# ut-amrl/vision_slam_frontend

Measured on AMD Instinct MI355X. Metric: stereo frames/s (640x480, 2000 kp/frame), higher is better.
Workload: dtype u8

## Files before the change

include/vsf.h:

```cpp
#ifndef VSF_H_
#define VSF_H_

#include <stddef.h>
#include <stdint.h>

#ifdef __cplusplus
extern "C" {
#endif

#define VSF_VERSION 2
#define VSF_DESC_BYTES 32
#define VSF_MAX_LEVELS 64

typedef enum {
  VSF_OK = 0,
  VSF_ERR_INVALID_ARG = 1,
  VSF_ERR_CAPACITY = 2,
  VSF_ERR_HIP = 3,
  VSF_ERR_UNSUPPORTED = 4,
  VSF_ERR_NO_DEVICE = 5
} vsf_status;

typedef struct {
  float x, y;
// ... 12 lines not shown
typedef struct {
  int32_t nfeatures;
  float scale_factor;
  int32_t nlevels;
  int32_t edge_threshold;
  int32_t first_level;
  int32_t wta_k;
  int32_t score_type;
  int32_t patch_size;
  int32_t fast_threshold;
  int32_t blur_sse2;
  int32_t fast_detector_threshold;
  int32_t fast_detector_nms;
  uint32_t ratio_num;
  uint32_t ratio_shift;
  int32_t width, height;
  int32_t max_images;
  int32_t max_keypoints;
  int32_t residual_order;
} vsf_params;

typedef struct vsf_ctx vsf_ctx;

vsf_status vsf_params_default(vsf_params* p, int width, int height, int max_images);
vsf_status vsf_params_set_ratio(vsf_params* p, float nn_match_ratio);

vsf_status vsf_create(const vsf_params* p, int device, vsf_ctx** out);
void vsf_destroy(vsf_ctx* ctx);
const char* vsf_status_string(vsf_status s);
int vsf_last_hip_error(const vsf_ctx* ctx);
vsf_status vsf_get_params(const vsf_ctx* ctx, vsf_params* out);
vsf_status vsf_set_stream(vsf_ctx* ctx, void* hip_stream);
vsf_status vsf_set_lanes(vsf_ctx* ctx, int lanes);
vsf_status vsf_set_pipeline(vsf_ctx* ctx, int on);
vsf_status vsf_set_input_event(vsf_ctx* ctx, void* hip_event);
vsf_status vsf_set_blur_overlap(vsf_ctx* ctx, int on);
vsf_status vsf_set_fast_resident(vsf_ctx* ctx, int waves);
vsf_status vsf_get_fast_resident(const vsf_ctx* ctx, int* waves);
vsf_status vsf_tune_fast_resident(vsf_ctx* ctx, const uint8_t* d_imgs, int n_images, size_t image_stride,
                                  size_t row_stride, vsf_keypoint* d_kp, uint8_t* d_desc, int32_t* d_counts,
                                  int samples, float* ms_grid, float* ms_resident);
typedef enum {
  VSF_OPT_FAST_BOTH_MAX = 0,
  VSF_OPT_SELECT_WIDE = 1,
  VSF_OPT_PYRAMID_FEW = 2,
  VSF_OPT_PYRAMID_CHAIN = 3,
  VSF_OPT_PYRAMID_ROWS = 4,
  VSF_OPT_SELECT_BIG_CLASS = 5,
  VSF_OPT_PIPE_AFTER_FAST = 6,
  VSF_OPT_PIPE_PRIORITY = 7,
  VSF_OPT_OBSERVE_THREAD = 8,
  VSF_OPT_PYRAMID_TAIL_MIN = 9,
  VSF_OPT_OBSERVE_COPY_THREAD = 10,
  VSF_OPT_COUNT = 11
} vsf_option;
vsf_status vsf_set_option(vsf_ctx* ctx, int option, int value);
vsf_status vsf_get_option(const vsf_ctx* ctx, int option, int* value);
vsf_status vsf_sync(vsf_ctx* ctx);
vsf_status vsf_reserve(vsf_ctx* ctx, int n_frames, int n_pairs);

vsf_status vsf_level_info(const vsf_ctx* ctx, int level, int* w, int* h, float* scale, int* nfeatures);

#define VSF_COMM_ID_BYTES 128
typedef struct vsf_comm vsf_comm;
vsf_status vsf_comm_unique_id(uint8_t* id);
vsf_status vsf_comm_create(vsf_ctx* ctx, const uint8_t* id, int rank, int world, vsf_comm** out);
void vsf_comm_destroy(vsf_comm* comm);
vsf_status vsf_comm_info(const vsf_comm* comm, int* rank, int* world, int* rccl_version);
vsf_status vsf_allgather_dev(vsf_ctx* ctx, vsf_comm* comm, const void* d_send, void* d_recv, size_t bytes_per_rank);
vsf_status vsf_gather_payload_dev(vsf_ctx* ctx, vsf_comm* comm, const uint8_t* d_send, size_t bytes, uint8_t* d_recv,
                                  size_t recv_stride, int root);


vsf_status vsf_extract(vsf_ctx* ctx, const uint8_t* img, int w, int h, size_t stride, vsf_keypoint* kp_out,
                       uint8_t* desc_out, int cap, int* n_out);
vsf_status vsf_extract_pair(vsf_ctx* ctx, const uint8_t* img0, const uint8_t* img1, int w, int h, size_t stride,
                            vsf_keypoint* kp0, uint8_t* desc0, int* n0, vsf_keypoint* kp1, uint8_t* desc1, int* n1,
                            int cap);
vsf_status vsf_fast_detect(vsf_ctx* ctx, const uint8_t* img, int w, int h, size_t stride, int threshold, int nms,
                           vsf_keypoint* kp_out, int cap, int* n_out);
vsf_status vsf_knn2_hamming(vsf_ctx* ctx, const uint8_t* q, int nq, const uint8_t* t, int nt, int32_t* idx2,
                            int32_t* dist2);
vsf_status vsf_get_matches(vsf_ctx* ctx, const uint8_t* q, int nq, const uint8_t* t, int nt, vsf_dmatch* out,
                           int cap, int* n_out);

vsf_status vsf_get_matches_multi(vsf_ctx* ctx, const uint8_t* const* q, const int* nq, int n_sets, const uint8_t* t,
                                 int nt, vsf_dmatch* out, int cap_per_set, int* n_out);


vsf_status vsf_extract_batch_dev(vsf_ctx* ctx, const uint8_t* d_imgs, int n_images, size_t image_stride,
                                 size_t row_stride, vsf_keypoint* d_kp, uint8_t* d_desc, int32_t* d_counts);
vsf_status vsf_match_batch_dev(vsf_ctx* ctx, const uint8_t* d_desc, const int32_t* d_counts, size_t set_stride,
                               const int32_t* d_q_set, const int32_t* d_t_set, int n_pairs, int32_t* d_idx2,
                               int32_t* d_dist2, vsf_dmatch* d_matches, int32_t* d_nmatches);
vsf_status vsf_stereo_batch_dev(vsf_ctx* ctx, const uint8_t* d_imgs, int n_frames, size_t image_stride,
                                size_t row_stride, vsf_keypoint* d_kp, uint8_t* d_desc, int32_t* d_counts,
                                vsf_dmatch* d_matches, int32_t* d_nmatches);


vsf_status vsf_remove_ambig_stereo_batch_dev(vsf_ctx* ctx, const vsf_keypoint* d_kp, const uint8_t* d_desc,
                                             const vsf_dmatch* d_matches, const int32_t* d_nmatches, int n_frames,
                                             const float* F, float thr_in, const float* d_thr_override,
                                             float* d_means, float* d_thr, vsf_keypoint* d_kp_out,
                                             uint8_t* d_desc_out, int32_t* d_counts_out);
vsf_status vsf_feature_matches_batch_dev(vsf_ctx* ctx, const uint8_t* d_desc, const int32_t* d_counts,
                                         size_t set_stride, const int32_t* d_q_set, const int32_t* d_t_set,
                                         int n_pairs, float best_percent, uint64_t* d_pairs, int32_t* d_npairs);
// ... 96 lines not shown
```

vision_slam_frontend_amd/capi.py:

```python
from __future__ import annotations

import ctypes as C
from pathlib import Path

import numpy as np

_PKG = Path(__file__).resolve().parent
LIB_PATH = _PKG / "libvsf_hip.so"

KEYPOINT_DTYPE = np.dtype([("x", "<f4"), ("y", "<f4"), ("size", "<f4"), ("angle", "<f4"), ("response", "<f4"),
                           ("octave", "<i4"), ("class_id", "<i4")])
DMATCH_DTYPE = np.dtype([("queryIdx", "<i4"), ("trainIdx", "<i4"), ("imgIdx", "<i4"), ("distance", "<f4")])
VISION_FEATURE_DTYPE = np.dtype([("feature_idx", "<u8"), ("pixel", "<f4", (2,)), ("point3d", "<f4", (3,))])
FEATURE_MATCH_DTYPE = np.dtype([("feature_idx_initial", "<u8"), ("feature_idx_current", "<u8")])
assert VISION_FEATURE_DTYPE.itemsize == 28 and FEATURE_MATCH_DTYPE.itemsize == 16
DESC_BYTES = 32
PAYLOAD_MAGIC = 0x31465356

VSF_OK, VSF_ERR_INVALID_ARG, VSF_ERR_CAPACITY, VSF_ERR_HIP, VSF_ERR_UNSUPPORTED, VSF_ERR_NO_DEVICE = range(6)

EXPORTS = [
    "vsf_params_default", "vsf_params_set_ratio", "vsf_create", "vsf_destroy", "vsf_status_string",
    "vsf_last_hip_error", "vsf_get_params", "vsf_set_stream", "vsf_sync", "vsf_level_info", "vsf_extract",
    "vsf_fast_detect", "vsf_knn2_hamming", "vsf_get_matches", "vsf_extract_pair", "vsf_get_matches_multi", "vsf_extract_batch_dev", "vsf_match_batch_dev",
    "vsf_stereo_batch_dev", "vsf_set_lanes", "vsf_set_pipeline", "vsf_set_blur_overlap", "vsf_set_fast_resident", "vsf_get_fast_resident", "vsf_remove_ambig_stereo_batch_dev", "vsf_feature_matches_batch_dev", "vsf_bayer_bg_to_gray_batch_dev", "vsf_debug_level_image", "vsf_debug_fast_candidates", "vsf_debug_level_keypoints",
    "vsf_algorithmic_bytes_per_image", "vsf_pyramid_pixels", "vsf_profile_enable", "vsf_profile_read",
    "vsf_stage_name", "vsf_debug_retain_best", "vsf_debug_sort_trim", "vsf_stereo_residuals_batch_dev", "vsf_stereo_thresholds_dev",
    "vsf_stereo_filter_batch_dev", "vsf_vision_features_batch_dev", "vsf_packed_outputs_capacity",
    "vsf_pack_outputs_dev", "vsf_observe_capacity", "vsf_observe_stereo", "vsf_observe_submit", "vsf_observe_collect", "vsf_observe_reset",
    "vsf_observe_configure", "vsf_observe_collect_view", "vsf_observe_stats", "vsf_observe_poll", "vsf_debug_jpeg_serial",
    "vsf_jpeg_decode_gray_batch", "vsf_png_decode_gray_batch", "vsf_imdecode_gray_batch", "vsf_tune_fast_resident", "vsf_set_option", "vsf_get_option", "vsf_debug_inject_hip_error", "vsf_comm_unique_id", "vsf_comm_create", "vsf_comm_destroy", "vsf_comm_info",
    "vsf_allgather_dev", "vsf_gather_payload_dev", "vsf_reserve", "vsf_set_input_event",
]
(OPT_FAST_BOTH_MAX, OPT_SELECT_WIDE, OPT_PYRAMID_FEW, OPT_PYRAMID_CHAIN, OPT_PYRAMID_ROWS, OPT_SELECT_BIG_CLASS,
 OPT_PIPE_AFTER_FAST, OPT_PIPE_PRIORITY, OPT_OBSERVE_THREAD, OPT_PYRAMID_TAIL_MIN, OPT_OBSERVE_COPY_THREAD) = range(11)
STAGE_COUNT = 8


class VsfParams(C.Structure):
    _fields_ = [("nfeatures", C.c_int32), ("scale_factor", C.c_float), ("nlevels", C.c_int32),
                ("edge_threshold", C.c_int32), ("first_level", C.c_int32), ("wta_k", C.c_int32),
                ("score_type", C.c_int32), ("patch_size", C.c_int32), ("fast_threshold", C.c_int32),
                ("blur_sse2", C.c_int32), ("fast_detector_threshold", C.c_int32), ("fast_detector_nms", C.c_int32),
                ("ratio_num", C.c_uint32), ("ratio_shift", C.c_uint32), ("width", C.c_int32), ("height", C.c_int32),
                ("max_images", C.c_int32), ("max_keypoints", C.c_int32), ("residual_order", C.c_int32)]


class VsfCalibration(C.Structure):
    _fields_ = [("projection_left", C.c_float * 12), ("projection_right", C.c_float * 12),
                ("camera_matrix_left", C.c_float * 9), ("distortion_left", C.c_float * 5),
                ("fundamental", C.c_float * 9), ("triangulate_rows", C.c_int32)]

    def set(self, name: str, values) -> "VsfCalibration":
        arr = getattr(self, name)
        v = np.ascontiguousarray(values, np.float32).reshape(-1)
        assert len(v) == len(arr), name
        for i, x in enumerate(v):
            arr[i] = float(x)
        return self

    def get(self, name: str) -> np.ndarray:
        return np.array(list(getattr(self, name)), np.float32)


class VsfError(RuntimeError):
    def __init__(self, status: int, where: str, hip: int = 0):
        self.status = status
        msg = "%s: %s" % (where, lib().vsf_status_string(status).decode())
        if status == VSF_ERR_HIP:
            msg += " (hipError %d)" % hip
        super().__init__(msg)


_lib = None


def lib() -> C.CDLL:
    global _lib
    if _lib is None:
        if not LIB_PATH.exists():
            raise ImportError("%s is missing: run `python -c 'import __graft_entry__ as g; g.build()'` "
                              "(hipcc --offload-arch=gfx950). The product has no CPU fallback." % LIB_PATH)
        L = C.CDLL(str(LIB_PATH))
        vp, i32, sz, pp = C.c_void_p, C.c_int, C.c_size_t, C.POINTER(VsfParams)
        ip = C.POINTER(C.c_int)
        L.vsf_params_default.argtypes = [pp, i32, i32, i32]
        L.vsf_params_set_ratio.argtypes = [pp, C.c_float]
        L.vsf_create.argtypes = [pp, i32, C.POINTER(vp)]
# ... 515 lines not shown
```

vision_slam_frontend_amd/csrc/vsf_api.hip:

```cpp
#include <algorithm>
#include <cfloat>
#include <climits>
#include <cmath>
#include <cstdio>
#include <cstring>
#include <new>
#include <vector>

#include "vsf_ctx.h"

using namespace vsfi;

thread_local int vsf_tls_hip_error = 0;

namespace vsfi {

vsf_status alloc_devset(vsf_ctx* ctx, const Geometry& G, DevSet* ds, bool orb, int n_images) {
  VSF_HIP(upload(&ds->levels, G.levels));
  VSF_HIP(upload(&ds->units, G.units));
  VSF_HIP(upload(&ds->blur_mma_units, G.blur_mma_units));
  VSF_HIP(upload(&ds->blur_mma_units_small, G.blur_mma_units_small));
  VSF_HIP(upload(&ds->blur_tcol, G.blur_tcol));
  VSF_HIP(upload(&ds->blur_tv, G.blur_tv));
  VSF_HIP(upload(&ds->ic_table, build_ic_table()));
// ... 135 lines not shown
  return VSF_OK;
}

void prof_fold(vsf_ctx* ctx) {
  for (size_t i = 0; i < ctx->ev_used; i++) {
    float ms = 0.f;
    if (hipEventElapsedTime(&ms, ctx->ev_pool[2 * i], ctx->ev_pool[2 * i + 1]) == hipSuccess) {
      ctx->prof_ms[ctx->ev_stage[i]] += ms;
      ctx->prof_launches[ctx->ev_stage[i]] += ctx->ev_launches[i];
    }
  }
  ctx->ev_used = 0;
}

void sync_all_streams(vsf_ctx* ctx) {
  if (ctx->stream) vsf_note(hipStreamSynchronize(ctx->stream));
  if (ctx->own_stream && ctx->own_stream != ctx->stream) vsf_note(hipStreamSynchronize(ctx->own_stream));
  if (ctx->aux_stream) vsf_note(hipStreamSynchronize(ctx->aux_stream));
  if (ctx->pipe_stream) vsf_note(hipStreamSynchronize(ctx->pipe_stream));
  if (ctx->blur_stream) vsf_note(hipStreamSynchronize(ctx->blur_stream));
  for (int i = 1; i < ctx->side.n; i++)
    if (ctx->side.stream[i]) vsf_note(hipStreamSynchronize(ctx->side.stream[i]));
  if (ctx->ob.copy_stream) vsf_note(hipStreamSynchronize(ctx->ob.copy_stream));
  if (ctx->ob.tail_stream) vsf_note(hipStreamSynchronize(ctx->ob.tail_stream));
}

VsfDev shifted(const VsfDev& d, const VsfGeom& g, int i0) {
  VsfDev o = d;
  const size_t i = (size_t)i0;
  if (o.pyr) o.pyr += i * g.pyr_bytes;
  if (o.blur) o.blur += i * g.pyr_bytes;
  o.cand += i * g.cand_entries;
  o.rowstart += i * (size_t)g.nunits * VSF_FAST_RS_STRIDE;
  if (o.scratch) o.scratch += i * 6 * g.cand_entries;
  if (o.lvlkp) o.lvlkp += i * g.lvlkp_entries;
  if (o.lvl_count) o.lvl_count += i * g.nlevels;
  return o;
}

void extract_on(vsf_ctx* ctx, hipStream_t st, const VsfImages& im_all, int i0, int n, vsf_keypoint* d_kp,
                uint8_t* d_desc, int32_t* d_counts, bool inputs_complete, const VsfSideStream* own_side, int32_t* status,
                int status_stride) {
  const VsfGeom& g = ctx->orb.g;
  VsfDev d = shifted(ctx->dorb.d, g, i0);
  if (status) {
    d.status = status;
    d.status_stride = status_stride;
  }
  VsfImages im = im_all;
  im.base += (size_t)i0 * im.image_stride;
  im.n = n;
  const size_t K = (size_t)ctx->p.max_keypoints;
  const bool pipe = ctx->pipeline && inputs_complete && ctx->lanes == 1 && st == ctx->stream && i0 == 0;
  if (pipe) {
    const int buf = ctx->pyr_flip;
    d.pyr = buf ? ctx->pyr_alt : ctx->dorb.d.pyr;
    hipStream_t ps = ctx->pipe_stream ? ctx->pipe_stream : ctx->aux_stream;
    if (ctx->pyr_free_valid[buf]) vsf_note(hipStreamWaitEvent(ps, ctx->ev_pyr_free[buf], 0));
    if (ctx->fast_done_valid && ctx->tuning.pipe_after_fast) vsf_note(hipStreamWaitEvent(ps, ctx->ev_fast_done, 0));
    if (ctx->ingest_done_valid) vsf_note(hipStreamWaitEvent(ps, ctx->ev_ingest_done, 0));
    if (ctx->input_event) vsf_note(hipStreamWaitEvent(ps, ctx->input_event, 0));
    {
      StageTimer t(ctx, ps, VSF_STAGE_PYRAMID, g.nlevels - 1);
      vsf_launch_pyramid(d, g, ctx->orb.levels.data(), im, ps, nullptr);
    }
    vsf_note(hipEventRecord(ctx->ev_pyr_done, ps));
    vsf_note(hipStreamWaitEvent(st, ctx->ev_pyr_done, 0));
  } else {
    StageTimer t(ctx, st, VSF_STAGE_PYRAMID, g.nlevels - 1);
    vsf_launch_pyramid(d, g, ctx->orb.levels.data(), im, st, own_side ? own_side : (ctx->lanes == 1 ? &ctx->side : nullptr));
  }
  ctx->last_pyr = d.pyr - (size_t)i0 * g.pyr_bytes;
  const bool beside_ok = ctx->blur_overlap && im.n >= 32 && ctx->blur_stream;
  int resident = 0;
  if (beside_ok && ctx->lanes == 1 && st == ctx->stream && i0 == 0 && !own_side) {
    if (ctx->fast_force >= 0)
      resident = ctx->fast_force;
    else if (ctx->fast_resident >= 0)
      resident = ctx->fast_resident;
    else if (ctx->fast_tune.n == im.n && ctx->fast_tune.choice > 0)
      resident = ctx->fast_tune.choice;
  }
  const bool blur_beside = beside_ok;
  auto launch_blur = [&](hipStream_t bs) {
    StageTimer t(ctx, bs, VSF_STAGE_BLUR, 1);
    if (im.n >= 32)
      vsf_launch_blur_mma(d, g, im, ctx->dorb.blur_mma_units, (int)ctx->orb.blur_mma_units.size(), ctx->dorb.blur_tcol,
                          ctx->dorb.blur_tv, ctx->orb.blur_bias, bs);
    else
      vsf_launch_blur_mma(d, g, im, ctx->dorb.blur_mma_units_small, (int)ctx->orb.blur_mma_units_small.size(),
                          ctx->dorb.blur_tcol, ctx->dorb.blur_tv, ctx->orb.blur_bias, bs);
  };
  auto fork_blur = [&]() {
    vsf_note(hipEventRecord(ctx->ev_blur_fork, st));
    vsf_note(hipStreamWaitEvent(ctx->blur_stream, ctx->ev_blur_fork, 0));
    launch_blur(ctx->blur_stream);
    vsf_note(hipEventRecord(ctx->ev_blur_done, ctx->blur_stream));
  };
  if (blur_beside) fork_blur();
  {
    StageTimer t(ctx, st, VSF_STAGE_FAST, 1);
    vsf_launch_fast(d, g, im, ctx->p.fast_threshold, 1, st, blur_beside ? resident : 0, ctx->n_cus, ctx->fast_cells);
  }
  if (pipe) {
    vsf_note(hipEventRecord(ctx->ev_fast_done, st));
    ctx->fast_done_valid = true;
  }
  {
    StageTimer t(ctx, st, VSF_STAGE_SELECT, 1);
    vsf_launch_select(d, g, ctx->orb.levels.data(), im, st);
  }
  if (blur_beside)
    vsf_note(hipStreamWaitEvent(st, ctx->ev_blur_done, 0));
  else
    launch_blur(st);
  {
    StageTimer t(ctx, st, VSF_STAGE_DESCRIBE, 1);
    vsf_launch_describe(d, g, im, ctx->p.max_keypoints, d_kp + i0 * K, d_desc + i0 * K * VSF_DESC_BYTES, d_counts + i0,
                        st);
  }
  if (pipe) {
    const int buf = ctx->pyr_flip;
    vsf_note(hipEventRecord(ctx->ev_pyr_free[buf], st));
    ctx->pyr_free_valid[buf] = true;
    ctx->pyr_flip ^= 1;
  }
}

void match_on(vsf_ctx* ctx, hipStream_t st, const uint8_t* d_desc, const int32_t* d_counts, size_t set_stride,
              const int32_t* d_q_set, const int32_t* d_t_set, int p0, int n, int32_t* d_idx2, int32_t* d_dist2,
              vsf_dmatch* d_matches, int32_t* d_nmatches, int32_t* status) {
  const int rows = ctx->p.max_keypoints;
  const size_t R = (size_t)rows;
  const uint8_t* desc = d_desc;
  const int32_t* counts = d_counts;
  if (!d_q_set) {
    desc += (size_t)(2 * p0) * set_stride;
    counts += 2 * p0;
  }
  int32_t* idx2 = d_idx2 + (size_t)p0 * R * 2;
  int32_t* dist2 = d_dist2 + (size_t)p0 * R * 2;
  {
    StageTimer t(ctx, st, VSF_STAGE_KNN2, 1);
    vsf_launch_knn2(desc, counts, set_stride, d_q_set ? d_q_set + p0 : nullptr, d_t_set ? d_t_set + p0 : nullptr, n,
                    rows, idx2, dist2, st);
  }
  {
    StageTimer t(ctx, st, VSF_STAGE_RATIO, 1);
    vsf_launch_ratio_compact(counts, d_q_set ? d_q_set + p0 : nullptr, d_t_set ? d_t_set + p0 : nullptr, n, rows, idx2,
                             dist2, ctx->p.ratio_num, ctx->p.ratio_shift, d_matches + (size_t)p0 * R, d_nmatches + p0,
                             status ? status : ctx->d_status, st);
  }
}

vsf_status fork_lane(vsf_ctx* ctx) {
  VSF_HIP(hipEventRecord(ctx->ev_fork, ctx->stream));
  VSF_HIP(hipStreamWaitEvent(ctx->aux_stream, ctx->ev_fork, 0));
  return VSF_OK;
}
vsf_status join_lane(vsf_ctx* ctx) {
  VSF_HIP(hipEventRecord(ctx->ev_join, ctx->aux_stream));
  VSF_HIP(hipStreamWaitEvent(ctx->stream, ctx->ev_join, 0));
  return VSF_OK;
}

vsf_status extract_async(vsf_ctx* ctx, const VsfImages& im, vsf_keypoint* d_kp, uint8_t* d_desc, int32_t* d_counts,
                         bool inputs_complete) {
  vsf_status st = run_chunked(ctx, im.n, [&](hipStream_t s, int i0, int n) {
    extract_on(ctx, s, im, i0, n, d_kp, d_desc, d_counts, inputs_complete);
  });
  if (st != VSF_OK) return st;
  ctx->last_images = im;
  ctx->last_valid = true;
  VSF_STICKY();
  return VSF_OK;
}

vsf_status ensure_pipeline_buffers(vsf_ctx* ctx) {
  if (ctx->pyr_alt) return VSF_OK;
  VSF_HIP(hipMalloc((void**)&ctx->pyr_alt, (size_t)ctx->p.max_images * ctx->orb.g.pyr_bytes));
  VSF_HIP(hipEventCreateWithFlags(&ctx->ev_pyr_done, hipEventDisableTiming));
  VSF_HIP(hipEventCreateWithFlags(&ctx->ev_fast_done, hipEventDisableTiming));
  for (hipEvent_t& e : ctx->ev_pyr_free) VSF_HIP(hipEventCreateWithFlags(&e, hipEventDisableTiming));
  return VSF_OK;
}

}

hipStream_t vsf_ctx_stream(const vsf_ctx* ctx) { return ctx->stream; }
int vsf_ctx_device(const vsf_ctx* ctx) { return ctx->device; }
void vsf_ctx_set_last_error(vsf_ctx* ctx, int code) { ctx->last_hip = code; }
void vsf_ctx_absorb_noted_error(vsf_ctx* ctx) {
  if (ctx->pending_hip == 0) ctx->pending_hip = vsf_tls_hip_error;
  vsf_tls_hip_error = 0;
}

extern "C" {

vsf_status vsf_params_default(vsf_params* p, int width, int height, int max_images) {
  if (!p) return VSF_ERR_INVALID_ARG;
  std::memset(p, 0, sizeof(*p));
  p->nfeatures = 10000;
  p->scale_factor = 1.04f;
  p->nlevels = 50;
  p->edge_threshold = 31;
  p->first_level = 0;
  p->wta_k = 2;
  p->score_type = 0;
  p->patch_size = 31;
  p->fast_threshold = 20;
  p->blur_sse2 = 1;
  p->residual_order = 0;
  p->fast_detector_threshold = 10;
  p->fast_detector_nms = 1;
  p->width = width;
  p->height = height;
  p->max_images = max_images;
  p->max_keypoints = 0;
  return vsf_params_set_ratio(p, 0.6f);
}

vsf_status vsf_params_set_ratio(vsf_params* p, float nn_match_ratio) {
  if (!p || !(nn_match_ratio > 0.f) || !(nn_match_ratio < 256.f)) return VSF_ERR_INVALID_ARG;
  double r = (double)nn_match_ratio;
  uint32_t shift = 0;
  while (r != std::floor(r) && shift < 31) {
    r *= 2.0;
    ++shift;
  }
  if (r != std::floor(r) || r >= 4294967296.0) return VSF_ERR_INVALID_ARG;
  p->ratio_num = (uint32_t)r;
  p->ratio_shift = shift;
  return VSF_OK;
// ... 64 lines not shown
  if (hipMemset(ctx->d_status, 0, 4 * sizeof(int32_t)) != hipSuccess) return fail(VSF_ERR_HIP);
  {
    int per_block = 0, per_cu = 0;
    if (hipDeviceGetAttribute(&per_block, hipDeviceAttributeMaxSharedMemoryPerBlock, device) != hipSuccess) per_block = 0;
    if (hipDeviceGetAttribute(&per_cu, hipDeviceAttributeMaxSharedMemoryPerMultiprocessor, device) != hipSuccess) per_cu = 0;
    int limit = std::min(std::max(std::max(per_block, per_cu), 64 * 1024), 160 * 1024);
    if (vsf_prepare_sort_kernels(limit) != hipSuccess) {
      (void)hipGetLastError();
      limit = 64 * 1024;
    }
    ctx->tuning.lds_limit = limit;
    if (vsf_prepare_pyramid_kernels(limit) != hipSuccess) {
      (void)hipGetLastError();
      ctx->tuning.pyramid_chain = 0;
    }
    if (vsf_prepare_jpeg_kernels(limit) != hipSuccess) {
      (void)hipGetLastError();
      ctx->tuning.jpeg_serial = 1;
    }
  }
  if (hipMalloc((void**)&ctx->fast_cells, 2 * sizeof(uint32_t)) != hipSuccess) return fail(VSF_ERR_HIP);
  if (hipHostMalloc((void**)&ctx->h_status, sizeof(int32_t), hipHostMallocDefault) != hipSuccess)
    return fail(VSF_ERR_HIP);
  vsf_status st = alloc_devset(ctx, ctx->orb, &ctx->dorb, true, ctx->p.max_images);
  if (st != VSF_OK) return fail(st);
  ctx->st_img_pitch = (size_t)align_up(ctx->p.width, 64);
  ctx->st_img_stride = ctx->st_img_pitch * (size_t)ctx->p.height;
  const size_t n = (size_t)ctx->p.max_images, K = (size_t)ctx->p.max_keypoints;
  if (hipMalloc((void**)&ctx->st_img, n * ctx->st_img_stride) != hipSuccess ||
      hipMalloc((void**)&ctx->st_kp, n * K * sizeof(vsf_keypoint)) != hipSuccess ||
      hipMalloc((void**)&ctx->st_desc, n * K * VSF_DESC_BYTES) != hipSuccess ||
      hipMalloc((void**)&ctx->st_counts, n * sizeof(int32_t)) != hipSuccess)
    return fail(VSF_ERR_HIP);
  if (reserve_scratch(ctx, std::max(1, ctx->p.max_images / 2), std::max(1, ctx->p.max_images / 2)) != VSF_OK)
    return fail(VSF_ERR_HIP);
  if (hipDeviceSynchronize() != hipSuccess) return fail(VSF_ERR_HIP);
  *out = ctx;
  return VSF_OK;
}

void vsf_destroy(vsf_ctx* ctx) {
  if (!ctx) return;
  hipSetDevice(ctx->device);
  stop_observe_threads(ctx);
  sync_all_streams(ctx);
  vsf_tls_hip_error = 0;
  if (ctx->ev_pyr_done) {
    hipEventDestroy(ctx->ev_pyr_done);
    hipEventDestroy(ctx->ev_fast_done);
    for (hipEvent_t e : ctx->ev_pyr_free) hipEventDestroy(e);
  }
  if (ctx->ev_ingest_done) hipEventDestroy(ctx->ev_ingest_done);
  hipFree(ctx->pyr_alt);
  free_devset(&ctx->dorb);
  free_devset(&ctx->dfast);
  hipFree(ctx->d_status);
  hipFree(ctx->fast_cells);
  for (hipEvent_t e : ctx->fast_tune.ev)
    if (e) hipEventDestroy(e);
  if (ctx->h_status) hipHostFree(ctx->h_status);
  hipFree(ctx->st_img);
  hipFree(ctx->st_kp);
  hipFree(ctx->st_desc);
  hipFree(ctx->st_counts);
  hipFree(ctx->m_idx2);
  hipFree(ctx->m_dist2);
  hipFree(ctx->f_residual);
  hipFree(ctx->t_matches);
  hipFree(ctx->t_nmatches);
  hipFree(ctx->t_sortkeys);
  free_observe(ctx);
  hipFree(ctx->jp_flags);
  hipFree(ctx->png_filtered);
  hipFree(ctx->png_file_status);
  hipFree(ctx->jp_clean);
  hipFree(ctx->jp_coef);
  for (int i = 0; i < 2; i++) {
    if (ctx->jp_host[i]) hipHostFree(ctx->jp_host[i]);
    hipFree(ctx->jp_dev[i]);
    if (ctx->jp_copied[i]) hipEventDestroy(ctx->jp_copied[i]);
  }
  free_retired(ctx);
  hipFree(ctx->v_pairs);
  hipFree(ctx->v_npairs);
  hipFree(ctx->v_sets);
  hipFree(ctx->pk_offsets);
  hipFree(ctx->mm_desc);
  hipFree(ctx->mm_counts);
  hipFree(ctx->mm_matches);
  hipFree(ctx->mm_nmatches);
  hipFree(ctx->mh_desc);
  hipFree(ctx->mh_counts);
  hipFree(ctx->mh_matches);
  hipFree(ctx->mh_nmatches);
  for (hipEvent_t e : ctx->ev_pool) hipEventDestroy(e);
  if (ctx->ev_fork) hipEventDestroy(ctx->ev_fork);
  if (ctx->ev_join) hipEventDestroy(ctx->ev_join);
  if (ctx->side.fork) hipEventDestroy(ctx->side.fork);
  for (int i = 0; i < VSF_SIDE_STREAMS; i++) {
    if (ctx->side.join[i]) hipEventDestroy(ctx->side.join[i]);
    if (i > 0 && ctx->side.stream[i]) {
      hipStreamSynchronize(ctx->side.stream[i]);
      hipStreamDestroy(ctx->side.stream[i]);
    }
  }
  if (ctx->aux_stream) hipStreamDestroy(ctx->aux_stream);
// ... 17 lines not shown
  VsfErrorScope scope_(ctx);
  if (!ctx) return VSF_ERR_INVALID_ARG;
  VSF_HIP(hipStreamSynchronize(ctx->stream));
  prof_fold(ctx);
  ctx->stream = hip_stream ? (hipStream_t)hip_stream : ctx->own_stream;
  return VSF_OK;
}

vsf_status vsf_set_lanes(vsf_ctx* ctx, int lanes) {
  VsfErrorScope scope_(ctx);
  if (!ctx || lanes < 1 || lanes > 2) return VSF_ERR_INVALID_ARG;
  VSF_HIP(hipStreamSynchronize(ctx->stream));
  ctx->lanes = lanes;
  return VSF_OK;
}

vsf_status vsf_set_blur_overlap(vsf_ctx* ctx, int on) {
  VsfErrorScope scope_(ctx);
  if (!ctx) return VSF_ERR_INVALID_ARG;
  VSF_HIP(hipStreamSynchronize(ctx->stream));
  ctx->blur_overlap = on ? 1 : 0;
  return VSF_OK;
}

vsf_status vsf_set_fast_resident(vsf_ctx* ctx, int waves) {
  VsfErrorScope scope_(ctx);
  if (!ctx || waves < -1 || waves == 1 || waves > 4) return VSF_ERR_INVALID_ARG;
  VSF_HIP(hipStreamSynchronize(ctx->stream));
  ctx->fast_resident = waves;
  return VSF_OK;
}

vsf_status vsf_get_fast_resident(const vsf_ctx* ctx, int* waves) {
  if (!ctx || !waves) return VSF_ERR_INVALID_ARG;
  *waves = ctx->fast_resident >= 0 ? ctx->fast_resident : std::max(ctx->fast_tune.choice, 0);
  return VSF_OK;
}

vsf_status vsf_set_option(vsf_ctx* ctx, int option, int value) {
  VsfErrorScope scope_(ctx);
  if (!ctx || option < 0 || option >= VSF_OPT_COUNT) return VSF_ERR_INVALID_ARG;
  VSF_HIP(hipStreamSynchronize(ctx->stream));
  VsfTuning& t = ctx->tuning;
  switch (option) {
    case VSF_OPT_FAST_BOTH_MAX:
      if (value < 0) return VSF_ERR_INVALID_ARG;
      t.fast_both_max = value;
      break;
    case VSF_OPT_SELECT_WIDE: t.select_wide = value != 0; break;
    case VSF_OPT_SELECT_BIG_CLASS: t.select_big_class = value != 0; break;
    case VSF_OPT_PIPE_AFTER_FAST: t.pipe_after_fast = value != 0; break;
    case VSF_OPT_OBSERVE_THREAD: t.observe_thread = value != 0; break;
    case VSF_OPT_OBSERVE_COPY_THREAD: t.observe_copy_thread = value != 0; break;
    case VSF_OPT_PIPE_PRIORITY:
      if (value < -1 || value > 1) return VSF_ERR_INVALID_ARG;
      t.pipe_priority = value;
      break;
    case VSF_OPT_PYRAMID_FEW:
      if (value < 0) return VSF_ERR_INVALID_ARG;
      t.pyramid_few = value;
      break;
    case VSF_OPT_PYRAMID_CHAIN:
      if (value < 0 || value > 64) return VSF_ERR_INVALID_ARG;
      if (value > 0 && t.lds_limit < 160 * 1024 - 2048) return VSF_ERR_UNSUPPORTED;
      t.pyramid_chain = value;
      break;
    case VSF_OPT_PYRAMID_ROWS:
      if (value < 1) return VSF_ERR_INVALID_ARG;
      t.pyramid_rows = value;
      break;
    case VSF_OPT_PYRAMID_TAIL_MIN:
      if (value < 0) return VSF_ERR_INVALID_ARG;
      t.pyramid_tail_min = value;
      break;
    default: return VSF_ERR_INVALID_ARG;
  }
  return VSF_OK;
}

vsf_status vsf_get_option(const vsf_ctx* ctx, int option, int* value) {
  if (!ctx || !value) return VSF_ERR_INVALID_ARG;
  const VsfTuning& t = ctx->tuning;
  switch (option) {
    case VSF_OPT_FAST_BOTH_MAX: *value = t.fast_both_max; break;
    case VSF_OPT_SELECT_WIDE: *value = t.select_wide; break;
    case VSF_OPT_SELECT_BIG_CLASS: *value = t.select_big_class; break;
    case VSF_OPT_PIPE_AFTER_FAST: *value = t.pipe_after_fast; break;
    case VSF_OPT_OBSERVE_THREAD: *value = t.observe_thread; break;
    case VSF_OPT_OBSERVE_COPY_THREAD: *value = t.observe_copy_thread; break;
    case VSF_OPT_PIPE_PRIORITY: *value = t.pipe_priority; break;
    case VSF_OPT_PYRAMID_FEW: *value = t.pyramid_few; break;
    case VSF_OPT_PYRAMID_CHAIN: *value = t.pyramid_chain; break;
    case VSF_OPT_PYRAMID_ROWS: *value = t.pyramid_rows; break;
    case VSF_OPT_PYRAMID_TAIL_MIN: *value = t.pyramid_tail_min; break;
    default: return VSF_ERR_INVALID_ARG;
  }
  return VSF_OK;
}

vsf_status vsf_set_pipeline(vsf_ctx* ctx, int on) {
  VsfErrorScope scope_(ctx);
  if (!ctx) return VSF_ERR_INVALID_ARG;
  VSF_HIP(hipSetDevice(ctx->device));
  VSF_HIP(hipStreamSynchronize(ctx->stream));
  VSF_HIP(hipStreamSynchronize(ctx->aux_stream));
  if (ctx->pipe_stream) VSF_HIP(hipStreamSynchronize(ctx->pipe_stream));
  if (on && ctx->tuning.pipe_priority != ctx->pipe_stream_priority) {
    if (ctx->pipe_stream) VSF_HIP(hipStreamDestroy(ctx->pipe_stream));
    ctx->pipe_stream = nullptr;
    ctx->pipe_stream_priority = 0;
    if (ctx->tuning.pipe_priority != 0) {
      int least = 0, greatest = 0;
      VSF_HIP(hipDeviceGetStreamPriorityRange(&least, &greatest));
      VSF_HIP(hipStreamCreateWithPriority(&ctx->pipe_stream, hipStreamNonBlocking,
                                          ctx->tuning.pipe_priority > 0 ? least : greatest));
      ctx->pipe_stream_priority = ctx->tuning.pipe_priority;
    }
  }
  if (on) {
    const vsf_status st = ensure_pipeline_buffers(ctx);
    if (st != VSF_OK) return st;
  }
  ctx->pipeline = on != 0;
  ctx->pyr_free_valid[0] = ctx->pyr_free_valid[1] = false;
  ctx->fast_done_valid = false;
  return VSF_OK;
}

vsf_status vsf_sync(vsf_ctx* ctx) {
  VsfErrorScope scope_(ctx);
  if (!ctx) return VSF_ERR_INVALID_ARG;
  const vsf_status st = check_status_word(ctx);
  if (!ctx->retired.empty() || !ctx->retired_host.empty()) {
    sync_all_streams(ctx);
    free_retired(ctx);
  }
  return st;
}

vsf_status vsf_set_input_event(vsf_ctx* ctx, void* hip_event) {
  VsfErrorScope scope_(ctx);
  if (!ctx) return VSF_ERR_INVALID_ARG;
// ... 45 lines not shown
```

vision_slam_frontend_amd/csrc/vsf_ctx.h:

```cpp
#ifndef VSF_CTX_H_
#define VSF_CTX_H_

#include <cstddef>
#include <cstdint>
#include <vector>

#include "vsf_internal.h"

namespace vsfi {

inline int align_up(int v, int a) { return (v + a - 1) / a * a; }

struct Geometry {
  VsfGeom g{};
  std::vector<VsfLevel> levels;
  std::vector<uint32_t> units;
  std::vector<VsfTap> xt, yt;
  std::vector<uint32_t> blur_mma_units, blur_mma_units_small;
  std::vector<uint4> blur_tcol, blur_tv;
  int blur_bias = 0;
};

struct DevSet {
  VsfDev d{};
  VsfLevel* levels = nullptr;
  uint32_t* units = nullptr;
  uint32_t* blur_mma_units = nullptr;
  uint32_t* blur_mma_units_small = nullptr;
  uint4* blur_tcol = nullptr;
  uint4* blur_tv = nullptr;
  uint2* ic_table = nullptr;
  bool ready = false;
};

bool build_geometry(const vsf_params& p, bool orb, bool nms, Geometry* out);
void gaussian_taps(int k[4]);
std::vector<uint2> build_ic_table();
std::vector<int> orb_umax(int patch_size);

}

struct vsf_ctx {
  vsf_params p{};
  int device = 0;
  int n_cus = 256;
  hipStream_t own_stream = nullptr, stream = nullptr;
  hipStream_t aux_stream = nullptr;
  hipEvent_t ev_fork = nullptr, ev_join = nullptr;
  hipStream_t blur_stream = nullptr;
  hipEvent_t ev_blur_fork = nullptr, ev_blur_done = nullptr;
  VsfSideStream side{};
  bool pipeline = false;
  hipStream_t pipe_stream = nullptr;
  int pipe_stream_priority = 0;
  uint8_t* pyr_alt = nullptr;
  int pyr_flip = 0;
  hipEvent_t ev_pyr_done = nullptr, ev_pyr_free[2] = {nullptr, nullptr}, ev_fast_done = nullptr;
  bool pyr_free_valid[2] = {false, false}, fast_done_valid = false;
  hipEvent_t ev_ingest_done = nullptr;
  bool ingest_done_valid = false;
  hipEvent_t input_event = nullptr;
  const uint8_t* last_pyr = nullptr;
  int lanes = 1;
  int blur_overlap = 1;
  int fast_resident = -1;
  int fast_force = -1;
  VsfTuning tuning;
  int last_hip = 0;
  int pending_hip = 0;
  vsfi::Geometry orb, fast;
  vsfi::DevSet dorb, dfast;
  int32_t* d_status = nullptr;
  uint32_t* fast_cells = nullptr;
  struct FastTune {
    int n = 0, choice = -1;
    hipEvent_t ev[2] = {nullptr, nullptr};
  } fast_tune;
  int32_t* h_status = nullptr;
  uint8_t* st_img = nullptr;
  size_t st_img_pitch = 0, st_img_stride = 0;
  vsf_keypoint* st_kp = nullptr;
  uint8_t* st_desc = nullptr;
  int32_t* st_counts = nullptr;
  int32_t* m_idx2 = nullptr;
  int32_t* m_dist2 = nullptr;
  int m_pairs = 0, m_rows = 0;
  float* f_residual = nullptr;
  int f_frames = 0;
  vsf_dmatch* t_matches = nullptr;
  int32_t* t_nmatches = nullptr;
  void* t_sortkeys = nullptr;
  int t_pairs = 0;
  uint64_t* v_pairs = nullptr;
  int32_t* v_npairs = nullptr;
  int32_t* v_sets = nullptr;
  int v_frames = 0;
  uint32_t* pk_offsets = nullptr;
  int pk_entries = 0;
  std::vector<void*> retired;
  std::vector<void*> retired_host;
  static constexpr int kObserveBatchSlots = 4;
  struct ObserveLauncher;
  struct ObserveCopyHelper;
  struct ObserveBatchMeta;
  struct ObserveBatch {
    uint8_t* d_img = nullptr;
    vsf_keypoint* kp_raw = nullptr;
    uint8_t* desc_raw = nullptr;
    int32_t* counts_raw = nullptr;
    vsf_dmatch* matches = nullptr;
    int32_t* nmatches = nullptr;
    int32_t* status = nullptr;
    ObserveBatchMeta* h_meta = nullptr;
    hipEvent_t ev_uploaded = nullptr, ev_extracted = nullptr, ev_done = nullptr;
    bool used = false;
// ... 213 lines not shown
```

vision_slam_frontend_amd/csrc/vsf_debug.hip:

```cpp
#include <algorithm>
#include <cfloat>
#include <climits>
#include <cmath>
#include <cstdio>
#include <cstring>
#include <new>
#include <vector>

#include "vsf_ctx.h"

using namespace vsfi;

extern "C" {

vsf_status vsf_debug_inject_hip_error(vsf_ctx* ctx, int code) {
  VsfErrorScope scope_(ctx);
  if (!ctx || code <= 0) return VSF_ERR_INVALID_ARG;
  vsf_note((hipError_t)code);
  return VSF_OK;
}

vsf_status vsf_debug_jpeg_serial(vsf_ctx* ctx, int on) {
  VsfErrorScope scope_(ctx);
  if (!ctx) return VSF_ERR_INVALID_ARG;
// ... 76 lines not shown
  if (!ctx || !matches || !pairs_out || !counts_out || n_lists < 1 || n < 0 || n > ctx->p.max_keypoints)
    return VSF_ERR_INVALID_ARG;
  VSF_HIP(hipSetDevice(ctx->device));
  const size_t K = (size_t)ctx->p.max_keypoints;
  vsf_dmatch* dm = nullptr;
  int32_t *dn = nullptr, *dc = nullptr;
  uint64_t* dp = nullptr;
  void* dscratch = nullptr;
  hipError_t e = hipMalloc((void**)&dm, (size_t)n_lists * K * sizeof(vsf_dmatch));
  if (e == hipSuccess) e = hipMalloc((void**)&dn, (size_t)n_lists * sizeof(int32_t));
  if (e == hipSuccess) e = hipMalloc((void**)&dc, (size_t)n_lists * sizeof(int32_t));
  if (e == hipSuccess) e = hipMalloc((void**)&dp, (size_t)n_lists * K * 2 * sizeof(uint64_t));
  if (e == hipSuccess) e = hipMalloc(&dscratch, (size_t)n_lists * K * 8);
  std::vector<int32_t> hn((size_t)n_lists, n);
  if (e == hipSuccess) e = hipMemcpy(dn, hn.data(), hn.size() * sizeof(int32_t), hipMemcpyHostToDevice);
  for (int i = 0; i < n_lists && e == hipSuccess && n > 0; i++)
    e = hipMemcpy(dm + (size_t)i * K, matches + (size_t)i * n, (size_t)n * sizeof(vsf_dmatch), hipMemcpyHostToDevice);
  if (e == hipSuccess) {
    vsf_launch_sort_trim(dm, dn, n_lists, (int)K, best_percent, nullptr, dscratch, dp, dc, ctx->stream, serial != 0,
                         ctx->tuning.lds_limit);
    e = hipStreamSynchronize(ctx->stream);
  }
  if (e == hipSuccess) e = hipMemcpy(counts_out, dc, (size_t)n_lists * sizeof(int32_t), hipMemcpyDeviceToHost);
  for (int i = 0; i < n_lists && e == hipSuccess && n > 0; i++)
    e = hipMemcpy(pairs_out + (size_t)i * n * 2, dp + (size_t)i * K * 2, (size_t)n * 2 * sizeof(uint64_t),
                  hipMemcpyDeviceToHost);
  hipFree(dm);
  hipFree(dn);
  hipFree(dc);
  hipFree(dp);
  hipFree(dscratch);
  if (e != hipSuccess) {
    ctx->last_hip = (int)e;
    return VSF_ERR_HIP;
  }
  return VSF_OK;
}

vsf_status vsf_debug_level_image(vsf_ctx* ctx, int image, int level, int blurred, uint8_t* out, size_t ostride) {
  VsfErrorScope scope_(ctx);
  if (!ctx || !out || !ctx->last_valid || image < 0 || image >= ctx->last_images.n || level < 0 ||
      level >= ctx->orb.g.nlevels)
    return VSF_ERR_INVALID_ARG;
  const VsfLevel& L = ctx->orb.levels[level];
  if (ostride < (size_t)L.w) return VSF_ERR_INVALID_ARG;
  VSF_HIP(hipSetDevice(ctx->device));
  VSF_HIP(hipStreamSynchronize(ctx->stream));
  const uint8_t* src;
  size_t pitch;
  if (!blurred && level == 0) {
    src = ctx->last_images.base + (size_t)image * ctx->last_images.image_stride;
    pitch = ctx->last_images.row_stride;
  } else {
    src = (blurred ? ctx->dorb.d.blur : (ctx->last_pyr ? ctx->last_pyr : ctx->dorb.d.pyr)) +
          (size_t)image * ctx->orb.g.pyr_bytes + L.offset;
    pitch = (size_t)L.pitch;
  }
  if (blurred) {
    std::vector<uint8_t> tiled((size_t)L.pitch * align_up(L.h, 8));
    VSF_HIP(hipMemcpy(tiled.data(), src, tiled.size(), hipMemcpyDeviceToHost));
    for (int y = 0; y < L.h; y++)
      for (int x = 0; x < L.w; x++) out[(size_t)y * ostride + x] = tiled[VSF_BLUR_TILE_OFFSET(L.pitch, x, y)];
    return VSF_OK;
  }
  VSF_HIP(hipMemcpy2D(out, ostride, src, pitch, (size_t)L.w, (size_t)L.h, hipMemcpyDeviceToHost));
  return VSF_OK;
}

vsf_status vsf_debug_fast_candidates(vsf_ctx* ctx, int image, int level, vsf_keypoint* kp_out, int cap, int* n_out) {
  VsfErrorScope scope_(ctx);
  if (!ctx || !n_out || !ctx->last_valid || image < 0 || image >= ctx->last_images.n || level < 0 ||
      level >= ctx->orb.g.nlevels)
    return VSF_ERR_INVALID_ARG;
  VSF_HIP(hipSetDevice(ctx->device));
  VSF_HIP(hipStreamSynchronize(ctx->stream));
  const VsfLevel& L = ctx->orb.levels[level];
  const VsfGeom& g = ctx->orb.g;
  const int nu = L.nstrips * L.nbands;
  int n = 0;
  if (nu > 0) {
    std::vector<uint16_t> rs((size_t)nu * VSF_FAST_RS_STRIDE);
    VSF_HIP(hipMemcpy(rs.data(), ctx->dorb.d.rowstart + ((size_t)image * g.nunits + L.unit0) * VSF_FAST_RS_STRIDE,
                      rs.size() * sizeof(uint16_t), hipMemcpyDeviceToHost));
    std::vector<uint32_t> seg((size_t)nu * L.seg_cap);
    VSF_HIP(hipMemcpy(seg.data(), ctx->dorb.d.cand + (size_t)image * g.cand_entries + L.cand_offset,
                      seg.size() * sizeof(uint32_t), hipMemcpyDeviceToHost));
    for (int row = 0; row < L.y_hi - L.y_lo; row++) {
      const int s = row / VSF_FAST_STRIP_ROWS, r = row % VSF_FAST_STRIP_ROWS;
      for (int b = 0; b < L.nbands; b++) {
        const int u = s * L.nbands + b;
        const uint16_t* urs = rs.data() + (size_t)u * VSF_FAST_RS_STRIDE;
        for (int e = urs[r]; e < urs[r + 1]; e++, n++) {
          if (n < cap && kp_out) {
            const uint32_t cd = seg[(size_t)u * L.seg_cap + e];
            kp_out[n] =
                vsf_keypoint{(float)VSF_CAND_X(cd), (float)VSF_CAND_Y(cd), 7.f, -1.f, (float)VSF_CAND_SCORE(cd), 0, -1};
          }
        }
      }
    }
  }
  *n_out = n;
  return VSF_OK;
}

vsf_status vsf_debug_level_keypoints(vsf_ctx* ctx, int image, int level, vsf_keypoint* kp_out, int cap, int* n_out) {
  VsfErrorScope scope_(ctx);
// ... 23 lines not shown
```

vision_slam_frontend_amd/csrc/vsf_internal.h:

```cpp
#ifndef VSF_INTERNAL_H_
#define VSF_INTERNAL_H_

#include <hip/hip_runtime.h>
#include <stdint.h>

#include <vector>

#include "../../include/vsf.h"

#define VSF_FAST_BAND_COLS 248
#define VSF_FAST_HALF_COLS 120
#define VSF_FAST_STRIP_ROWS 32
#define VSF_FAST_RS_STRIDE (VSF_FAST_STRIP_ROWS + 2)
#define VSF_BLUR_MMA_ROWS 26
#define VSF_BLUR_MMA_STEPS 16
#define VSF_BLUR_MMA_STEPS_SMALL 2
#define VSF_BLUR_TILE_OFFSET(pitch, x, y) \
  ((uint32_t)((y) >> 2) * (uint32_t)((pitch) * 4) + ((uint32_t)((x) >> 5) << 7) + ((uint32_t)((y) & 3) << 5) + (uint32_t)((x) & 31))
#define VSF_SORT_LDS_ROWS 4096
#define VSF_IC_ITEMS 320

struct VsfLevel {
  int32_t w, h;
  int32_t pitch;
// ... 6 lines not shown
  int32_t nbands, nstrips;
  int32_t unit0;
  uint32_t cand_offset;
  int32_t seg_cap;
  int32_t kp_offset;
  int32_t kp_cap;
  int32_t blur_vec_end;
  uint32_t xtab, ytab;
  int32_t resize_rows;
  int32_t resize_any8;
  uint32_t rscale_x[2], rscale_y[2];
  uint32_t blur_tcol;
};

struct VsfTap {
  uint16_t i0, i1;
  int16_t c0, c1;
};

#define VSF_CAND_PACK(x, y, s) (((uint32_t)(s) << 24) | ((uint32_t)(y) << 12) | (uint32_t)(x))
#define VSF_CAND_X(c) ((int)((c)&0xFFFu))
#define VSF_CAND_Y(c) ((int)(((c) >> 12) & 0xFFFu))
#define VSF_CAND_SCORE(c) ((int)((c) >> 24))

struct VsfLevelKp {
  uint32_t xy;
  float response;
  float angle;
  float ca, sb;
};

struct VsfGeom {
  int nlevels;
  int width, height;
  uint32_t pyr_bytes;
  uint32_t cand_entries;
  int nunits;
  int nwork_full, nwork_half;
  int lvlkp_entries;
  uint64_t pyramid_pixels;
};

struct VsfTuning {
  int fast_both_max = 16;
  int select_wide = 1;
  int pipe_priority = 0;
  int pipe_after_fast = 1;
  int select_big_class = 1;
  int jpeg_serial = 0;
  int pyramid_few = 16;
  int pyramid_chain = 8;
  int pyramid_rows = 6;
  int pyramid_tail_min = 0;
  int observe_copy_thread = 1;
  int observe_thread = 0;
  int lds_limit = 0;
};

extern thread_local int vsf_tls_hip_error;
inline void vsf_note(hipError_t e) {
  if (e != hipSuccess && vsf_tls_hip_error == 0) vsf_tls_hip_error = (int)e;
}
hipStream_t vsf_ctx_stream(const vsf_ctx* ctx);
int vsf_ctx_device(const vsf_ctx* ctx);
void vsf_ctx_set_last_error(vsf_ctx* ctx, int code);
constexpr int VSF_RCCL_ERROR_BASE = 10000;
void vsf_ctx_absorb_noted_error(vsf_ctx* ctx);
void vsf_ctx_enter(vsf_ctx* ctx);
struct VsfErrorScope {
  vsf_ctx* ctx;
  explicit VsfErrorScope(vsf_ctx* c, bool enter = true) : ctx(c) {
    if (ctx && enter) vsf_ctx_enter(ctx);
  }
  ~VsfErrorScope() {
    if (ctx && vsf_tls_hip_error != 0) vsf_ctx_absorb_noted_error(ctx);
  }
  VsfErrorScope(const VsfErrorScope&) = delete;
  VsfErrorScope& operator=(const VsfErrorScope&) = delete;
};
hipError_t vsf_prepare_sort_kernels(int lds_limit);
hipError_t vsf_prepare_pyramid_kernels(int lds_limit);
hipError_t vsf_prepare_jpeg_kernels(int lds_limit);

struct VsfDev {
  const VsfLevel* levels;
  const uint32_t* units;
  uint8_t* pyr;
  uint8_t* blur;
  uint32_t* cand;
  uint16_t* rowstart;
  uint32_t* scratch;
  VsfLevelKp* lvlkp;
  const uint2* ic_table;
  int32_t* lvl_count;
  int32_t* status;
  int status_stride;
  const VsfTuning* tune;
};

struct VsfImages {
  const uint8_t* base;
  size_t image_stride;
  size_t row_stride;
  int n;
};

// ... 133 lines not shown
```

Baseline: 41380.

## Launch blur on the pipeline chain right after pyramid with double-buffered blur

```diff
diff --git a/include/vsf.h b/include/vsf.h
--- a/include/vsf.h
+++ b/include/vsf.h
@@ -88,7 +88,8 @@
   VSF_OPT_OBSERVE_THREAD = 8,
   VSF_OPT_PYRAMID_TAIL_MIN = 9,
   VSF_OPT_OBSERVE_COPY_THREAD = 10,
-  VSF_OPT_COUNT = 11
+  VSF_OPT_BLUR_AFTER_PYRAMID = 11,
+  VSF_OPT_COUNT = 12
 } vsf_option;
 vsf_status vsf_set_option(vsf_ctx* ctx, int option, int value);
 vsf_status vsf_get_option(const vsf_ctx* ctx, int option, int* value);
diff --git a/vision_slam_frontend_amd/capi.py b/vision_slam_frontend_amd/capi.py
--- a/vision_slam_frontend_amd/capi.py
+++ b/vision_slam_frontend_amd/capi.py
@@ -33,7 +33,8 @@
     "vsf_allgather_dev", "vsf_gather_payload_dev", "vsf_reserve", "vsf_set_input_event",
 ]
 (OPT_FAST_BOTH_MAX, OPT_SELECT_WIDE, OPT_PYRAMID_FEW, OPT_PYRAMID_CHAIN, OPT_PYRAMID_ROWS, OPT_SELECT_BIG_CLASS,
- OPT_PIPE_AFTER_FAST, OPT_PIPE_PRIORITY, OPT_OBSERVE_THREAD, OPT_PYRAMID_TAIL_MIN, OPT_OBSERVE_COPY_THREAD) = range(11)
+ OPT_PIPE_AFTER_FAST, OPT_PIPE_PRIORITY, OPT_OBSERVE_THREAD, OPT_PYRAMID_TAIL_MIN, OPT_OBSERVE_COPY_THREAD,
+ OPT_BLUR_AFTER_PYRAMID) = range(12)
 STAGE_COUNT = 8
 
 
diff --git a/vision_slam_frontend_amd/csrc/vsf_api.hip b/vision_slam_frontend_amd/csrc/vsf_api.hip
--- a/vision_slam_frontend_amd/csrc/vsf_api.hip
+++ b/vision_slam_frontend_amd/csrc/vsf_api.hip
@@ -211,9 +211,19 @@
   im.n = n;
   const size_t K = (size_t)ctx->p.max_keypoints;
   const bool pipe = ctx->pipeline && inputs_complete && ctx->lanes == 1 && st == ctx->stream && i0 == 0;
+  auto launch_blur_mma = [&](hipStream_t bs) {
+    if (im.n >= 32)
+      vsf_launch_blur_mma(d, g, im, ctx->dorb.blur_mma_units, (int)ctx->orb.blur_mma_units.size(), ctx->dorb.blur_tcol,
+                          ctx->dorb.blur_tv, ctx->orb.blur_bias, bs);
+    else
+      vsf_launch_blur_mma(d, g, im, ctx->dorb.blur_mma_units_small, (int)ctx->orb.blur_mma_units_small.size(),
+                          ctx->dorb.blur_tcol, ctx->dorb.blur_tv, ctx->orb.blur_bias, bs);
+  };
+  const bool blur_on_chain = pipe && ctx->tuning.blur_after_pyramid && im.n >= 32 && ctx->blur_stream && ctx->blur_alt;
   if (pipe) {
     const int buf = ctx->pyr_flip;
     d.pyr = buf ? ctx->pyr_alt : ctx->dorb.d.pyr;
+    if (blur_on_chain) d.blur = buf ? ctx->blur_alt : ctx->dorb.d.blur;
     hipStream_t ps = ctx->pipe_stream ? ctx->pipe_stream : ctx->aux_stream;
     if (ctx->pyr_free_valid[buf]) vsf_note(hipStreamWaitEvent(ps, ctx->ev_pyr_free[buf], 0));
     if (ctx->fast_done_valid && ctx->tuning.pipe_after_fast) vsf_note(hipStreamWaitEvent(ps, ctx->ev_fast_done, 0));
@@ -225,11 +235,18 @@
     }
     vsf_note(hipEventRecord(ctx->ev_pyr_done, ps));
     vsf_note(hipStreamWaitEvent(st, ctx->ev_pyr_done, 0));
+    if (blur_on_chain) {
+      vsf_note(hipStreamWaitEvent(ctx->blur_stream, ctx->ev_pyr_done, 0));
+      StageTimer t(ctx, ctx->blur_stream, VSF_STAGE_BLUR, 1);
+      launch_blur_mma(ctx->blur_stream);
+      vsf_note(hipEventRecord(ctx->ev_blur_done, ctx->blur_stream));
+    }
   } else {
     StageTimer t(ctx, st, VSF_STAGE_PYRAMID, g.nlevels - 1);
     vsf_launch_pyramid(d, g, ctx->orb.levels.data(), im, st, own_side ? own_side : (ctx->lanes == 1 ? &ctx->side : nullptr));
   }
   ctx->last_pyr = d.pyr - (size_t)i0 * g.pyr_bytes;
+  ctx->last_blur = d.blur - (size_t)i0 * g.pyr_bytes;
   const bool beside_ok = ctx->blur_overlap && im.n >= 32 && ctx->blur_stream;
   int resident = 0;
   if (beside_ok && ctx->lanes == 1 && st == ctx->stream && i0 == 0 && !own_side) {
@@ -240,15 +257,10 @@
     else if (ctx->fast_tune.n == im.n && ctx->fast_tune.choice > 0)
       resident = ctx->fast_tune.choice;
   }
-  const bool blur_beside = beside_ok;
+  const bool blur_beside = beside_ok && !blur_on_chain;
   auto launch_blur = [&](hipStream_t bs) {
     StageTimer t(ctx, bs, VSF_STAGE_BLUR, 1);
-    if (im.n >= 32)
-      vsf_launch_blur_mma(d, g, im, ctx->dorb.blur_mma_units, (int)ctx->orb.blur_mma_units.size(), ctx->dorb.blur_tcol,
-                          ctx->dorb.blur_tv, ctx->orb.blur_bias, bs);
-    else
-      vsf_launch_blur_mma(d, g, im, ctx->dorb.blur_mma_units_small, (int)ctx->orb.blur_mma_units_small.size(),
-                          ctx->dorb.blur_tcol, ctx->dorb.blur_tv, ctx->orb.blur_bias, bs);
+    launch_blur_mma(bs);
   };
   auto fork_blur = [&]() {
     vsf_note(hipEventRecord(ctx->ev_blur_fork, st));
@@ -259,7 +271,7 @@
   if (blur_beside) fork_blur();
   {
     StageTimer t(ctx, st, VSF_STAGE_FAST, 1);
-    vsf_launch_fast(d, g, im, ctx->p.fast_threshold, 1, st, blur_beside ? resident : 0, ctx->n_cus, ctx->fast_cells);
+    vsf_launch_fast(d, g, im, ctx->p.fast_threshold, 1, st, beside_ok ? resident : 0, ctx->n_cus, ctx->fast_cells);
   }
   if (pipe) {
     vsf_note(hipEventRecord(ctx->ev_fast_done, st));
@@ -269,7 +281,7 @@
     StageTimer t(ctx, st, VSF_STAGE_SELECT, 1);
     vsf_launch_select(d, g, ctx->orb.levels.data(), im, st);
   }
-  if (blur_beside)
+  if (blur_beside || blur_on_chain)
     vsf_note(hipStreamWaitEvent(st, ctx->ev_blur_done, 0));
   else
     launch_blur(st);
@@ -336,8 +348,10 @@
 }
 
 vsf_status ensure_pipeline_buffers(vsf_ctx* ctx) {
-  if (ctx->pyr_alt) return VSF_OK;
-  VSF_HIP(hipMalloc((void**)&ctx->pyr_alt, (size_t)ctx->p.max_images * ctx->orb.g.pyr_bytes));
+  const size_t bytes = (size_t)ctx->p.max_images * ctx->orb.g.pyr_bytes;
+  if (!ctx->pyr_alt) VSF_HIP(hipMalloc((void**)&ctx->pyr_alt, bytes));
+  if (!ctx->blur_alt && ctx->tuning.blur_after_pyramid) VSF_HIP(hipMalloc((void**)&ctx->blur_alt, bytes));
+  if (ctx->ev_pyr_done) return VSF_OK;
   VSF_HIP(hipEventCreateWithFlags(&ctx->ev_pyr_done, hipEventDisableTiming));
   VSF_HIP(hipEventCreateWithFlags(&ctx->ev_fast_done, hipEventDisableTiming));
   for (hipEvent_t& e : ctx->ev_pyr_free) VSF_HIP(hipEventCreateWithFlags(&e, hipEventDisableTiming));
@@ -508,6 +522,7 @@
   }
   if (ctx->ev_ingest_done) hipEventDestroy(ctx->ev_ingest_done);
   hipFree(ctx->pyr_alt);
+  hipFree(ctx->blur_alt);
   free_devset(&ctx->dorb);
   free_devset(&ctx->dfast);
   hipFree(ctx->d_status);
@@ -631,6 +646,13 @@
     case VSF_OPT_PIPE_AFTER_FAST: t.pipe_after_fast = value != 0; break;
     case VSF_OPT_OBSERVE_THREAD: t.observe_thread = value != 0; break;
     case VSF_OPT_OBSERVE_COPY_THREAD: t.observe_copy_thread = value != 0; break;
+    case VSF_OPT_BLUR_AFTER_PYRAMID:
+      t.blur_after_pyramid = value != 0;
+      if (t.blur_after_pyramid && ctx->pipeline) {
+        const vsf_status st = ensure_pipeline_buffers(ctx);
+        if (st != VSF_OK) return st;
+      }
+      break;
     case VSF_OPT_PIPE_PRIORITY:
       if (value < -1 || value > 1) return VSF_ERR_INVALID_ARG;
       t.pipe_priority = value;
@@ -667,6 +689,7 @@
     case VSF_OPT_PIPE_AFTER_FAST: *value = t.pipe_after_fast; break;
     case VSF_OPT_OBSERVE_THREAD: *value = t.observe_thread; break;
     case VSF_OPT_OBSERVE_COPY_THREAD: *value = t.observe_copy_thread; break;
+    case VSF_OPT_BLUR_AFTER_PYRAMID: *value = t.blur_after_pyramid; break;
     case VSF_OPT_PIPE_PRIORITY: *value = t.pipe_priority; break;
     case VSF_OPT_PYRAMID_FEW: *value = t.pyramid_few; break;
     case VSF_OPT_PYRAMID_CHAIN: *value = t.pyramid_chain; break;
diff --git a/vision_slam_frontend_amd/csrc/vsf_ctx.h b/vision_slam_frontend_amd/csrc/vsf_ctx.h
--- a/vision_slam_frontend_amd/csrc/vsf_ctx.h
+++ b/vision_slam_frontend_amd/csrc/vsf_ctx.h
@@ -54,6 +54,7 @@
   hipStream_t pipe_stream = nullptr;
   int pipe_stream_priority = 0;
   uint8_t* pyr_alt = nullptr;
+  uint8_t* blur_alt = nullptr;
   int pyr_flip = 0;
   hipEvent_t ev_pyr_done = nullptr, ev_pyr_free[2] = {nullptr, nullptr}, ev_fast_done = nullptr;
   bool pyr_free_valid[2] = {false, false}, fast_done_valid = false;
@@ -61,6 +62,7 @@
   bool ingest_done_valid = false;
   hipEvent_t input_event = nullptr;
   const uint8_t* last_pyr = nullptr;
+  const uint8_t* last_blur = nullptr;
   int lanes = 1;
   int blur_overlap = 1;
   int fast_resident = -1;
diff --git a/vision_slam_frontend_amd/csrc/vsf_debug.hip b/vision_slam_frontend_amd/csrc/vsf_debug.hip
--- a/vision_slam_frontend_amd/csrc/vsf_debug.hip
+++ b/vision_slam_frontend_amd/csrc/vsf_debug.hip
@@ -152,7 +152,7 @@
     src = ctx->last_images.base + (size_t)image * ctx->last_images.image_stride;
     pitch = ctx->last_images.row_stride;
   } else {
-    src = (blurred ? ctx->dorb.d.blur : (ctx->last_pyr ? ctx->last_pyr : ctx->dorb.d.pyr)) +
+    src = (blurred ? (ctx->last_blur ? ctx->last_blur : ctx->dorb.d.blur) : (ctx->last_pyr ? ctx->last_pyr : ctx->dorb.d.pyr)) +
           (size_t)image * ctx->orb.g.pyr_bytes + L.offset;
     pitch = (size_t)L.pitch;
   }
diff --git a/vision_slam_frontend_amd/csrc/vsf_internal.h b/vision_slam_frontend_amd/csrc/vsf_internal.h
--- a/vision_slam_frontend_amd/csrc/vsf_internal.h
+++ b/vision_slam_frontend_amd/csrc/vsf_internal.h
@@ -82,6 +82,7 @@
   int pyramid_chain = 8;
   int pyramid_rows = 6;
   int pyramid_tail_min = 0;
+  int blur_after_pyramid = 1;
   int observe_copy_thread = 1;
   int observe_thread = 0;
   int lds_limit = 0;
```

Result: no change. 41720, median of 6 (+0.8%).
